# ESA-PRL/planning-path_planning

Measured on NVIDIA B200. Metric: plans_per_s, higher is better.
Workload: dtype f64

## Files before the change

### planning-path_planning_b200/csrc/dymu_fim.cu

```cuda
#include <cooperative_groups.h>
#include <stdlib.h>

#include "dymu_ctx.cuh"

namespace
{
constexpr int TILE = kTile;
static_assert(TILE == 32, "4 x 4 blocks of 8 x 8 cells");
constexpr int ROUNDS = 6;
constexpr int WARPS = 16;
constexpr int THREADS = 32 * WARPS;
constexpr int BX = TILE / 8;
constexpr int BY = TILE / 8;
constexpr int PITCH = TILE + 4;
constexpr int CPT = TILE * TILE / THREADS;
constexpr int MIN_CTAS = 2;
constexpr int SWEEP_CAP = 2 * TILE;
constexpr size_t SMEM = sizeof(double) * ((TILE + 2) * PITCH + TILE * PITCH);
constexpr size_t SMEM_ANISO = sizeof(double) * ((TILE + 2) * PITCH + 4 * TILE * PITCH);

constexpr uint32_t kHaloTop = 1u, kHaloBottom = 2u, kHaloLeft = 4u, kHaloRight = 8u, kFull = 16u,
                   kResume = 32u;

struct Params
{
    double* T;
    size_t slot_stride;
    const double* C;
    uint32_t pitch, rows, ntx, nty, nprob;
    uint32_t* list0;
    uint32_t* list1;
    uint32_t* list2;
    uint32_t* flag0;
    uint32_t* flag1;
    uint32_t* flag2;
    unsigned long long* key0;
    unsigned long long* key1;
    unsigned long long* key2;
    unsigned long long* gmin;
    uint32_t* dsave;
    unsigned long long* cta_trace;
    uint32_t cta_trace_phases;
    uint32_t* ctrl;
    unsigned long long* stats;
    int max_outer;
    int outer0;
    double band;
    unsigned long long* tmax;
    double* xout;
    size_t xld;
    uint32_t xnx, xny;
    int xminus1;
    const uint32_t* stop_flag;
    uint32_t stop_value;
    const double* A;
    size_t a_stride;
};
constexpr unsigned long long kExported = 0xFFFFFFFFFFFFFFFFull;

__device__ __forceinline__ uint32_t ld_volatile_u32(const uint32_t* p)
{
    return *reinterpret_cast<const volatile uint32_t*>(p);
}
__device__ __forceinline__ unsigned long long ld_volatile_u64(const unsigned long long* p)
{
    return *reinterpret_cast<const volatile unsigned long long*>(p);
}
__device__ __forceinline__ void smem_or(uint32_t* p, uint32_t v)
{
    asm volatile("red.shared.or.b32 [%0], %1;" ::"r"((uint32_t)__cvta_generic_to_shared(p)), "r"(v) : "memory");
}
constexpr unsigned long long kNoKey = 0xFFFFFFFFFFFFFFFFull;
__device__ __forceinline__ unsigned long long key_of(double v)
{
    return (unsigned long long)__double_as_longlong(v);
}

__device__ __noinline__ bool barrier_spin(const uint32_t* counter, uint32_t target,
                                          unsigned long long* abort_flag)
{
    uint32_t polls = 0;
    unsigned long long t0 = 0;
    while (ld_volatile_u32(counter) < target)
    {
        if ((++polls & 0x3FFFu) == 0)
        {
            if (ld_volatile_u64(abort_flag)) return false;
            unsigned long long now;
            asm volatile("mov.u64 %0, %%globaltimer;" : "=l"(now));
            if (t0 == 0) t0 = now;
            else if (now - t0 > 8000000000ull)
            {
                *abort_flag = 1ull;
                __threadfence();
                return false;
            }
        }
    }
    return true;
}

__device__ __forceinline__ bool grid_barrier(uint32_t* counter, uint32_t& phase, unsigned long long* abort_flag,
                                             uint32_t* ok)
{
    __syncthreads();
    if (threadIdx.x == 0)
    {
        __threadfence();
        uint32_t target = (phase + 1) * gridDim.x;
        atomicAdd(counter, 1u);
        *ok = barrier_spin(counter, target, abort_flag) ? 1u : 0u;
        __threadfence();
    }
    phase++;
    __syncthreads();
    return *ok != 0;
}

__device__ __forceinline__ void grid_barrier_arrive(uint32_t* counter, uint32_t phase, uint32_t* order)
{
    __syncthreads();
    if (threadIdx.x == 0)
    {
        __threadfence();
        *order = atomicAdd(counter, 1u) - phase * gridDim.x;
    }
}
__device__ __forceinline__ bool grid_barrier_wait(uint32_t* counter, uint32_t& phase, unsigned long long* abort_flag,
                                                  uint32_t* ok)
{
    if (threadIdx.x == 0)
    {
        uint32_t target = (phase + 1) * gridDim.x;
        *ok = barrier_spin(counter, target, abort_flag) ? 1u : 0u;
        __threadfence();
    }
    phase++;
    __syncthreads();
    return *ok != 0;
}

template <int MODE> __device__ __forceinline__ double outside_value()
{
    return MODE == 1 ? 0.0 : DYMU_INF;
}

__device__ __forceinline__ double min_nn(double a, double b)
{
    long long x = __double_as_longlong(a), y = __double_as_longlong(b);
    return __longlong_as_double(x < y ? x : y);
}
__device__ __forceinline__ double max_nn(double a, double b)
{
    long long x = __double_as_longlong(a), y = __double_as_longlong(b);
    return __longlong_as_double(x > y ? x : y);
}

template <int MODE>
__device__ __forceinline__ bool relax(double tc, double tl, double tr, double tu, double td,
                                      double c, double cc2 , double& out)
{
    if (MODE == 0)
    {
        const double Tx = min_nn(tl, tr), Ty = min_nn(td, tu);
        const double d = Tx - Ty;
        const bool two = fabs(d) < c;
        const double t2 = (Tx + Ty + dymu_sqrt_normal(cc2 - (d * d))) * 0.5;
        const double t1 = min_nn(Tx, Ty) + c;
        const double Tn = two ? t2 : t1;
        out = Tn;
        return Tn < tc;
    }
    else
    {
        const double Ry = max_nn(tu, td), Rx = max_nn(tl, tr);
        const double Sx = 1 - Rx, Sy = 1 - Ry;
        const double d = Sx - Sy;
        const bool target = c < DYMU_INF;
        const bool two = fabs(d) < c;
        double arg = (two && target) ? (2 * (c * c) - (d * d)) : 1.0;
        asm volatile("" : "+d"(arg));
        const double s2 = (Sx + Sy + dymu_sqrt_normal(arg)) / 2;
        const double s1 = fmin(Sx, Sy) + c;
        const double S = two ? s2 : s1;
        const double R = fmax(1 - S, 0.0);
        out = R;
        return target && (R > 0) && (R > tc);
    }
}

__device__ __forceinline__ double aniso_pair(double Th, double ah, double Tv, double av)
{
    const double d = Th - Tv;
    const double ah2 = ah * ah, av2 = av * av;
    const double s = ah2 + av2;
    const bool valid = (d > -ah) && (d < av) && (s < DYMU_INF);
    const double t = ((av2 * Th + ah2 * Tv) + (ah * av) * dymu_sqrt_normal(s - d * d)) / s;
    return valid ? t : DYMU_INF;
}

__device__ __forceinline__ bool relax_aniso(double tc, double txm, double txp, double tym, double typ,
                                            const double* ac, int ps, double& out)
{
    const double axm = ac[0], axp = ac[ps], aym = ac[2 * ps], ayp = ac[3 * ps];
    double Tn = min_nn(min_nn(txm + axm, txp + axp), min_nn(tym + aym, typ + ayp));
    Tn = min_nn(Tn, min_nn(aniso_pair(txm, axm, tym, aym), aniso_pair(txm, axm, typ, ayp)));
    Tn = min_nn(Tn, min_nn(aniso_pair(txp, axp, tym, aym), aniso_pair(txp, axp, typ, ayp)));
    out = Tn;
    return Tn < tc;
}

template <int MODE>
__global__ void __launch_bounds__(THREADS, MIN_CTAS) k_fim(Params p)
{
    constexpr int P = PITCH;
    extern __shared__ __align__(16) unsigned char smem_raw[];
    double* Ts = reinterpret_cast<double*>(smem_raw);
    double* Cs = Ts + (TILE + 2) * P;
    __shared__ uint32_t s_post[2][WARPS];
    __shared__ uint32_t s_m0;
    __shared__ uint32_t edge_mask;
    __shared__ uint32_t s_tile;
    __shared__ unsigned long long s_emin[5];
    __shared__ uint32_t s_tmax;
    __shared__ uint32_t s_xtile;
    __shared__ uint32_t s_xorder;
    __shared__ uint32_t s_bar_ok;

    const int tid = threadIdx.x, lane = tid & 31, warp = tid >> 5;
    const uint32_t tiles_per_prob = p.ntx * p.nty;
    constexpr int c_off = (TILE + 1) * P - 1;
    __shared__ uint2 s_wake[THREADS];
    double* cell1;
    int to_second;
    uint32_t my_bit;
    {
        const int lx = lane & 7, ly = lane >> 3;
        const bool upper_is_red = (lx & 1) == 0;
        to_second = upper_is_red ? P : -P;
        asm volatile("" : "+r"(to_second));
        const int bx = warp & 3, by = warp >> 2;
        int off = (by * 8 + 2 * ly + (upper_is_red ? 0 : 1) + 1) * P + bx * 8 + lx + 1;
        asm volatile("" : "+r"(off));
        cell1 = Ts + off;
        my_bit = 1u << warp;
        const uint32_t bitL = bx > 0 ? my_bit >> 1 : 0x40000u, bitR = bx < BX - 1 ? my_bit << 1 : 0x80000u;
        const uint32_t bitU = by > 0 ? my_bit >> 4 : 0x10000u, bitD = by < BY - 1 ? my_bit << 4 : 0x20000u;
        const uint32_t side = (lx == 0 ? bitL : 0u) | (lx == 7 ? bitR : 0u);
        const uint32_t w_upper = my_bit | side | (ly == 0 ? bitU : 0u);
        const uint32_t w_lower = my_bit | side | (ly == 3 ? bitD : 0u);
        s_wake[tid] = upper_is_red ? make_uint2(w_upper, w_lower) : make_uint2(w_lower, w_upper);
    }
    auto sel3 = [](uint32_t* a, uint32_t* b, uint32_t* c, int k) { return k == 0 ? a : (k == 1 ? b : c); };
    auto sel3k = [](unsigned long long* a, unsigned long long* b, unsigned long long* c, int k) {
        return k == 0 ? a : (k == 1 ? b : c);
    };
    auto deliver_tile = [&](uint32_t t) {
        const uint32_t ty = t / p.ntx, tx = t - ty * p.ntx;
#pragma unroll
        for (int k = 0; k < CPT; ++k)
        {
            const int e = tid + k * THREADS;
            const uint32_t gy = ty * TILE + e / TILE, gx = tx * TILE + e % TILE;
            if (gx < p.xnx && gy < p.xny)
            {
                double v = __ldcg(&p.T[(size_t)gy * p.pitch + gx]);
                if (p.xminus1 && v == DYMU_INF) v = -1.0;
                p.xout[(size_t)gy * p.xld + gx] = v;
            }
        }
    };
    uint32_t phase = 0;
    unsigned long long n_tiles = 0, n_visits = 0, n_deferred = 0, n_inner = 0;
    uint32_t n_written = 0;
#ifdef DYMU_FIM_PROFILE
    long long pc_fetch = 0, pc_load = 0, pc_sweep = 0, pc_store = 0, pc_barrier = 0, pc_t = clock64();
#define PC_MARK(acc) { long long now__ = clock64(); acc += now__ - pc_t; pc_t = now__; }
    unsigned long long tl_fetch = 0, tl_load = 0, tl_sweep = 0, tl_store = 0, tl_tiles = 0, tl_start = 0;
#define GT(var) { unsigned long long g__; asm volatile("mov.u64 %0, %%globaltimer;" : "=l"(g__)); var = g__; }
#else
#define PC_MARK(acc)
#endif
    int outer = p.outer0;
    bool converged = false;

    for (; outer < p.outer0 + p.max_outer; ++outer)
    {
        const int cur = outer % 3, nxt = (outer + 1) % 3, old = (outer + 2) % 3;
        const uint32_t n_active = ld_volatile_u32(&p.ctrl[kCtrlCount + cur]);
        if (n_active == 0)
        {
            converged = true;
            break;
        }
        if (p.stop_flag)
        {
            const uint32_t stop_at = ld_volatile_u32(&p.ctrl[kCtrlStopAt]);
            if (stop_at != 0 && stop_at <= (uint32_t)outer + 1u) break;
        }
#ifdef DYMU_FIM_PROFILE
        if (tid == 0) { GT(tl_start) tl_fetch = tl_load = tl_sweep = tl_store = tl_start; tl_tiles = 0; }
#endif
        uint32_t* list_cur = sel3(p.list0, p.list1, p.list2, cur);
        uint32_t* list_nxt = sel3(p.list0, p.list1, p.list2, nxt);
        uint32_t* flag_cur = sel3(p.flag0, p.flag1, p.flag2, cur);
        uint32_t* flag_nxt = sel3(p.flag0, p.flag1, p.flag2, nxt);
        unsigned long long* key_cur = sel3k(p.key0, p.key1, p.key2, cur);
        unsigned long long* key_nxt = sel3k(p.key0, p.key1, p.key2, nxt);
        unsigned long long limit = kNoKey;
        {
            const unsigned long long gm = ld_volatile_u64(&p.gmin[cur]);
            const double lim = __longlong_as_double((long long)gm) + p.band;
            if (gm != kNoKey && lim < DYMU_INF) limit = key_of(lim);
        }

        bool first_fetch = true;
        for (;;)
        {
            __syncthreads();
            if (tid == 0)
            {
                uint32_t t = 0xffffffffu;
                for (;;)
                {
                    uint32_t idx;
                    if (first_fetch)
                    {
                        idx = blockIdx.x;
                        first_fetch = false;
                    }
                    else
                    {
                        if (n_active <= gridDim.x) break;
                        idx = gridDim.x + atomicAdd(&p.ctrl[kCtrlCursor + cur], 1u);
                    }
                    if (idx >= n_active) break;
                    const uint32_t cand = ld_volatile_u32(&list_cur[idx]);
                    const unsigned long long k = ld_volatile_u64(&key_cur[cand]);
                    if (k <= limit)
                    {
                        t = cand;
                        break;
                    }
                    const uint32_t bits = ld_volatile_u32(&flag_cur[cand]);
                    flag_cur[cand] = 0;
                    key_cur[cand] = kNoKey;
                    atomicMin(&key_nxt[cand], k);
                    atomicMin(&p.gmin[nxt], k);
                    if (atomicOr(&flag_nxt[cand], bits) == 0)
                        list_nxt[atomicAdd(&p.ctrl[kCtrlCount + nxt], 1u)] = cand;
                    n_deferred++;
                }
                s_tile = t;
            }
            __syncthreads();
            PC_MARK(pc_fetch)
            const uint32_t tile_id = s_tile;
#ifdef DYMU_FIM_PROFILE
            if (tid == 0 && tile_id != 0xffffffffu && tl_tiles == 0) GT(tl_fetch)
#endif
            if (tile_id == 0xffffffffu) break;
            const uint32_t prob = tile_id / tiles_per_prob;
            const uint32_t trem = tile_id - prob * tiles_per_prob;
            const uint32_t ty = trem / p.ntx, tx = trem - ty * p.ntx;
            const uint32_t why = ld_volatile_u32(&flag_cur[tile_id]);
            double* Tg = p.T + (size_t)prob * p.slot_stride + (size_t)ty * TILE * p.pitch
                         + (size_t)tx * TILE;
            const double* Cg = p.C + (size_t)ty * TILE * p.pitch + (size_t)tx * TILE;

            static_assert(4 * TILE <= THREADS, "one halo cell per thread");
            double hv = outside_value<MODE>();
            int hslot = -1;
            if (tid < 4 * TILE)
            {
                const int side = tid / TILE, q = tid % TILE;
                const double* src = nullptr;
                if (side == 0)
                {
                    if (ty > 0) src = &Tg[-(ptrdiff_t)p.pitch + q];
                    hslot = q + 1;
                }
                else if (side == 1)
                {
                    if (ty + 1 < p.nty) src = &Tg[(size_t)TILE * p.pitch + q];
                    hslot = (TILE + 1) * P + q + 1;
                }
                else if (side == 2)
                {
                    if (tx > 0) src = &Tg[(size_t)q * p.pitch - 1];
                    hslot = (q + 1) * P;
                }
                else
                {
                    if (tx + 1 < p.ntx) src = &Tg[(size_t)q * p.pitch + TILE];
                    hslot = (q + 1) * P + TILE + 1;
                }
                if (src) hv = __ldcg(src);
            }
            double told[CPT];
#pragma unroll
            for (int k = 0; k < CPT; ++k)
            {
                int e = tid + k * THREADS;
                int y = e / TILE, x = e % TILE;
                double v = __ldcg(&Tg[(size_t)y * p.pitch + x]);
                told[k] = v;
                Ts[(y + 1) * P + x + 1] = v;
                if constexpr (MODE == 2)
                {
#pragma unroll
                    for (int q = 0; q < 4; ++q)
                        Cs[q * TILE * P + y * P + x] =
                            __ldg(&p.A[q * p.a_stride + (size_t)(ty * TILE + y) * p.pitch + tx * TILE + x]);
                }
                else
                    Cs[y * P + x] = __ldg(&Cg[(size_t)y * p.pitch + x]);
            }
            if (hslot >= 0) Ts[hslot] = hv;
            if (tid == 0)
            {
                uint32_t m0 = 0;
                if (why & kResume) m0 |= p.dsave[tile_id];
                if (why & kFull) m0 = 0xffffu;
                if (why & kHaloTop) m0 |= 0x000Fu;
                if (why & kHaloBottom) m0 |= 0xF000u;
                if (why & kHaloLeft) m0 |= 0x1111u;
                if (why & kHaloRight) m0 |= 0x8888u;
                s_m0 = m0;
                flag_cur[tile_id] = 0;
                key_cur[tile_id] = kNoKey;
            }
            if (tid == 0)
            {
                edge_mask = 0;
                s_tmax = 0;
            }
            if (tid < 5) s_emin[tid] = kNoKey;
            __syncthreads();
            PC_MARK(pc_load)
#ifdef DYMU_FIM_PROFILE
            if (tid == 0 && tl_tiles == 0) GT(tl_load)
#endif

            int it = 0;
            uint32_t visits = 0;
            uint32_t m = s_m0;
            uint32_t edges_acc = 0;
            const double cA = cell1[c_off], cB = cell1[to_second + c_off];
            const double qA = 2 * (cA * cA), qB = 2 * (cB * cB);
            auto sweep = [&](uint32_t* post) -> uint32_t {
                uint32_t contrib = 0;
                if (m & my_bit)
                {
                    double* a = cell1;
                    double* b = a + to_second;
                    uint2 wake = s_wake[tid];
                    asm volatile("" : "+r"(wake.x), "+r"(wake.y));
                    uint32_t woke = 0;
#pragma unroll
                    for (int round = 0; round < ROUNDS; ++round)
                    {
                        double tA = a[0];
                        const double lA = a[-1], rA = a[1], uA = a[-P], dA = a[P];
                        asm volatile("" : "+d"(tA));
                        double nA, nB;
                        bool chA;
                        if constexpr (MODE == 2)
                            chA = relax_aniso(tA, lA, rA, uA, dA, a + c_off, TILE * P, nA);
                        else
                            chA = relax<MODE>(tA, lA, rA, uA, dA, cA, qA, nA);
                        if (chA) a[0] = nA;
                        __syncwarp();
                        const double tB = b[0];
                        const double lB = b[-1], rB = b[1], uB = b[-P], dB = b[P];
                        bool chB;
                        if constexpr (MODE == 2)
                            chB = relax_aniso(tB, lB, rB, uB, dB, b + c_off, TILE * P, nB);
                        else
                            chB = relax<MODE>(tB, lB, rB, uB, dB, cB, qB, nB);
                        if (chB) b[0] = nB;
                        woke |= (chA ? wake.x : 0u) | (chB ? wake.y : 0u);
                        visits += 2;
                        if (round + 1 < ROUNDS)
                        {
                            if (!__any_sync(0xffffffffu, chA || chB)) break;
                        }
                    }
                    contrib = __reduce_or_sync(0xffffffffu, woke);
                }
                edges_acc |= contrib >> 16;
                if (lane == 0) post[warp] = contrib & 0xffffu;
                __syncthreads();
                ++it;
                return __reduce_or_sync(0xffffffffu, post[lane & (WARPS - 1)]);
            };
            for (;;)
            {
                if (m == 0 || it >= SWEEP_CAP) break;
                m = sweep(s_post[0]);
                if (m == 0 || it >= SWEEP_CAP) break;
                m = sweep(s_post[1]);
            }
            if (edges_acc && lane == 0) smem_or(&edge_mask, edges_acc);
            n_visits += visits;
            const int more = (m != 0);
            if (more && tid == 0) p.dsave[tile_id] = m;
            PC_MARK(pc_sweep)
#ifdef DYMU_FIM_PROFILE
            if (tid == 0 && tl_tiles == 0) GT(tl_sweep)
#endif

            uint32_t vmax = 0;
            {
                unsigned long long kmin[5] = {kNoKey, kNoKey, kNoKey, kNoKey, kNoKey};
                bool any = false;
#pragma unroll
                for (int k = 0; k < CPT; ++k)
                {
                    int e = tid + k * THREADS;
                    int y = e / TILE, x = e % TILE;
                    double v = Ts[(y + 1) * P + x + 1];
                    if (MODE != 1 && p.tmax && Cs[y * P + x] < DYMU_INF)
                        vmax = max(vmax, (uint32_t)(key_of(v) >> 32) + 1u);
                    if (v != told[k])
                    {
                        n_written++;
                        __stcg(&Tg[(size_t)y * p.pitch + x], v);
                        if (MODE != 1)
                        {
                            const unsigned long long kb = key_of(v);
                            any = true;
                            if (y == 0 && v < Ts[x + 1]) kmin[0] = min(kmin[0], kb);
                            if (y == TILE - 1 && v < Ts[(TILE + 1) * P + x + 1]) kmin[1] = min(kmin[1], kb);
                            if (x == 0 && v < Ts[(y + 1) * P]) kmin[2] = min(kmin[2], kb);
                            if (x == TILE - 1 && v < Ts[(y + 1) * P + TILE + 1]) kmin[3] = min(kmin[3], kb);
                            if (more) kmin[4] = min(kmin[4], kb);
                        }
                    }
                }
                if (MODE != 1 && __any_sync(0xffffffffu, any))
                {
#pragma unroll
                    for (int q = 0; q < 5; ++q)
                    {
                        const uint32_t hi = (uint32_t)(kmin[q] >> 32), lo = (uint32_t)kmin[q];
                        const uint32_t mhi = __reduce_min_sync(0xffffffffu, hi);
                        const uint32_t mlo = __reduce_min_sync(0xffffffffu, hi == mhi ? lo : 0xffffffffu);
                        const unsigned long long r = ((unsigned long long)mhi << 32) | mlo;
                        if (lane == 0 && r != kNoKey) atomicMin(&s_emin[q], r);
                    }
                }
            }
            if (MODE != 1 && p.tmax)
            {
                vmax = __reduce_max_sync(0xffffffffu, vmax);
                if (lane == 0 && vmax) atomicMax(&s_tmax, vmax);
            }
            __syncthreads();
            if (tid < 5)
            {
                uint32_t target = 0xffffffffu, bit = 0;
                uint32_t em = edge_mask;
                if (MODE != 1)
                    em = (s_emin[0] != kNoKey ? 1u : 0u) | (s_emin[1] != kNoKey ? 2u : 0u)
                         | (s_emin[2] != kNoKey ? 4u : 0u) | (s_emin[3] != kNoKey ? 8u : 0u);
                if (tid == 0 && (em & 1u) && ty > 0) { target = tile_id - p.ntx; bit = kHaloBottom; }
                if (tid == 1 && (em & 2u) && ty + 1 < p.nty) { target = tile_id + p.ntx; bit = kHaloTop; }
                if (tid == 2 && (em & 4u) && tx > 0) { target = tile_id - 1; bit = kHaloRight; }
                if (tid == 3 && (em & 8u) && tx + 1 < p.ntx) { target = tile_id + 1; bit = kHaloLeft; }
                if (tid == 4 && more) { target = tile_id; bit = kResume; }
                if (MODE != 1 && tid == 4 && p.tmax) p.tmax[tile_id] = (unsigned long long)s_tmax << 32;
                if (target != 0xffffffffu)
                {
                    unsigned long long kb = (MODE != 1) ? s_emin[tid] : 0ull;
                    if (kb == kNoKey) kb = 0ull;
                    atomicMin(&key_nxt[target], kb);
                    atomicMin(&p.gmin[nxt], kb);
                    if (atomicOr(&flag_nxt[target], bit) == 0)
                    {
                        uint32_t pos = atomicAdd(&p.ctrl[kCtrlCount + nxt], 1u);
                        list_nxt[pos] = target;
                    }
                }
            }
            n_tiles++;
            n_inner += (unsigned long long)it;
            PC_MARK(pc_store)
#ifdef DYMU_FIM_PROFILE
            if (tid == 0) { GT(tl_store) tl_tiles++; }
#endif
        }
        PC_MARK(pc_fetch)
#ifdef DYMU_FIM_PROFILE
        if (tid == 0 && p.cta_trace && (uint32_t)outer < p.cta_trace_phases)
        {
            unsigned long long tl_arrive; GT(tl_arrive)
            unsigned long long* o = p.cta_trace + ((size_t)outer * gridDim.x + blockIdx.x) * 8;
            o[0] = tl_start; o[1] = tl_fetch; o[2] = tl_load; o[3] = tl_sweep; o[4] = tl_store;
            o[5] = tl_arrive; o[6] = tl_tiles; o[7] = n_active;
        }
#endif
        if (blockIdx.x == 0 && tid == 0)
        {
            if (p.stop_flag && ld_volatile_u32(&p.ctrl[kCtrlStopAt]) == 0 && ld_volatile_u32(p.stop_flag) >= p.stop_value)
                p.ctrl[kCtrlStopAt] = (uint32_t)outer + 2u;
            p.ctrl[kCtrlCount + old] = 0;
            p.ctrl[kCtrlCursor + old] = 0;
            p.gmin[old] = kNoKey;
        }
        if (MODE != 1 && p.xout)
        {
            const unsigned long long gm = ld_volatile_u64(&p.gmin[cur]);
            grid_barrier_arrive(&p.ctrl[kCtrlBarrier], phase, &s_xorder);
            if (tid == 0) s_xtile = 0xffffffffu;
            __syncthreads();
            const uint32_t order = s_xorder, sharers = max(gridDim.x / 2u, 1u);
            if (order < sharers)
            {
                const uint32_t per = (tiles_per_prob + sharers - 1) / sharers;
                const uint32_t t_end = min((order + 1) * per, tiles_per_prob);
                for (uint32_t t = order * per + tid; t < t_end; t += THREADS)
                    if (ld_volatile_u64(&p.tmax[t]) < gm && atomicCAS(&s_xtile, 0xffffffffu, t) == 0xffffffffu)
                        p.tmax[t] = kExported;
                __syncthreads();
                const uint32_t xt = s_xtile;
                if (xt != 0xffffffffu)
                {
                    deliver_tile(xt);
                    if (tid == 0) atomicAdd(&p.stats[kStatDelivered], 1ull);
                }
            }
            if (!grid_barrier_wait(&p.ctrl[kCtrlBarrier], phase, &p.stats[kStatAbort], &s_bar_ok)) break;
        }
        else if (!grid_barrier(&p.ctrl[kCtrlBarrier], phase, &p.stats[kStatAbort], &s_bar_ok))
            break;
        PC_MARK(pc_barrier)
    }
#ifdef DYMU_FIM_PROFILE
    if (tid == 0)
    {
        atomicAdd(&p.stats[kStatCycFetch], (unsigned long long)pc_fetch);
        atomicAdd(&p.stats[kStatCycLoad], (unsigned long long)pc_load);
        atomicAdd(&p.stats[kStatCycSweep], (unsigned long long)pc_sweep);
        atomicAdd(&p.stats[kStatCycStore], (unsigned long long)pc_store);
        atomicAdd(&p.stats[kStatCycBarrier], (unsigned long long)pc_barrier);
    }
#endif

    if (lane == 0 && n_visits) atomicAdd(&p.stats[kStatVisits], n_visits);
    {
        const uint32_t w = __reduce_add_sync(0xffffffffu, n_written);
        if (lane == 0 && w) atomicAdd(&p.stats[kStatWritten], (unsigned long long)w);
    }
    if (tid == 0)
    {
        if (n_tiles) atomicAdd(&p.stats[kStatTiles], n_tiles);
        if (n_deferred) atomicAdd(&p.stats[kStatDeferred], n_deferred);
        if (n_inner) atomicAdd(&p.stats[kStatSweeps], n_inner);
        if (blockIdx.x == 0)
        {
            p.stats[kStatPhases] = (unsigned long long)(outer - p.outer0);
            p.stats[kStatConverged] = converged ? 1ull : 0ull;
        }
    }
}


__global__ void __launch_bounds__(512) k_deliver_rest(const double* T, uint32_t pitch, uint32_t ntx, uint32_t nty,
                                                      unsigned long long* tmax, double* xout, size_t xld,
                                                      uint32_t xnx, uint32_t xny, int xminus1,
                                                      unsigned long long* stats)
{
    if (ld_volatile_u64(&stats[kStatConverged]) == 0) return;
    const uint32_t total = ntx * nty;
    for (uint32_t t = blockIdx.x; t < total; t += gridDim.x)
    {
        if (ld_volatile_u64(&tmax[t]) == kExported) continue;
        const uint32_t ty = t / ntx, tx = t - ty * ntx;
        for (uint32_t e = threadIdx.x; e < TILE * TILE; e += blockDim.x)
        {
            const uint32_t gy = ty * TILE + e / TILE, gx = tx * TILE + e % TILE;
            if (gx < xnx && gy < xny)
            {
                double v = __ldcg(&T[(size_t)gy * pitch + gx]);
                if (xminus1 && v == DYMU_INF) v = -1.0;
                xout[(size_t)gy * xld + gx] = v;
            }
        }
    }
}

__global__ void k_seed(double* T, size_t slot_stride, uint32_t pitch, uint32_t ntx, uint32_t nty,
                       int tile, const uint32_t* goal_ij, uint32_t n, const uint8_t* obst, uint32_t* list0,
                       uint32_t* flag0, unsigned long long* key0, unsigned long long* gmin,
                       uint32_t* ctrl, unsigned long long* stats)
{
    if (blockIdx.x != 0 || threadIdx.x != 0) return;
    uint32_t n_seeded = 0;
    for (uint32_t q = 0; q < n; ++q)
    {
        uint32_t gi = goal_ij[2 * q], gj = goal_ij[2 * q + 1];
        if (obst && obst[(size_t)gj * pitch + gi])
        {
            stats[kStatGoalObstacle]++;
            continue;
        }
        T[(size_t)q * slot_stride + (size_t)gj * pitch + gi] = 0.0;
        uint32_t tile_id = q * ntx * nty + (gj / tile) * ntx + gi / tile;
        flag0[tile_id] = kFull;
        key0[tile_id] = 0ull;
        list0[n_seeded++] = tile_id;
    }
    ctrl[kCtrlCount] = n_seeded;
    if (n_seeded) gmin[0] = 0ull;
}

__global__ void k_seed_all(uint32_t n, uint32_t* list0, uint32_t* flag0, unsigned long long* key0,
                           unsigned long long* gmin, uint32_t* ctrl)
{
    uint32_t q = blockIdx.x * blockDim.x + threadIdx.x;
    if (q >= n) return;
    list0[q] = q;
    flag0[q] = kFull;
    key0[q] = 0ull;
    if (q == 0)
    {
        ctrl[kCtrlCount] = n;
        gmin[0] = 0ull;
    }
}

__global__ void k_seed_rows(uint32_t ntx, const uint32_t* tile_rows, uint32_t n_tile_rows, uint32_t* list0,
                            uint32_t* flag0, unsigned long long* key0, unsigned long long* gmin,
                            uint32_t* ctrl)
{
    uint32_t n = n_tile_rows * ntx;
    uint32_t q = blockIdx.x * blockDim.x + threadIdx.x;
    if (q >= n) return;
    uint32_t tile_id = tile_rows[q / ntx] * ntx + q % ntx;
    flag0[tile_id] = kFull;
    key0[tile_id] = 0ull;
    list0[q] = tile_id;
    if (q == 0)
    {
        ctrl[kCtrlCount] = n;
        gmin[0] = 0ull;
    }
}

__global__ void k_seed_rows_add(uint32_t ntx, const uint32_t* tile_rows, uint32_t n_tile_rows, uint32_t* list,
                                uint32_t* flag, unsigned long long* key, unsigned long long* gmin_cur,
                                uint32_t* count_cur, unsigned long long seed_key)
{
    uint32_t n = n_tile_rows * ntx;
    uint32_t q = blockIdx.x * blockDim.x + threadIdx.x;
    if (q >= n) return;
    uint32_t tile_id = tile_rows[q / ntx] * ntx + q % ntx;
    atomicMin(&key[tile_id], seed_key);
    if (atomicOr(&flag[tile_id], kFull) == 0) list[atomicAdd(count_cur, 1u)] = tile_id;
    if (q == 0) atomicMin(gmin_cur, seed_key);
}

__global__ void k_import_rows_min(double* T, uint32_t pitch, uint32_t nx, uint32_t j0, uint32_t n_rows,
                                  const double* src, int* changed, unsigned long long* min_lowered)
{
    size_t total = (size_t)nx * n_rows;
    size_t stride = (size_t)gridDim.x * blockDim.x;
    int any = 0;
    unsigned long long lowest = kNoKey;
    for (size_t k = (size_t)blockIdx.x * blockDim.x + threadIdx.x; k < total; k += stride)
    {
        uint32_t r = (uint32_t)(k / nx), i = (uint32_t)(k % nx);
        double v = src[k];
        double* t = &T[(size_t)(j0 + r) * pitch + i];
        if (v < *t)
        {
            *t = v;
            any = 1;
            lowest = min(lowest, key_of(v));
        }
    }
    if (__any_sync(0xffffffffu, any))
    {
        for (int o = 16; o > 0; o >>= 1) lowest = min(lowest, __shfl_xor_sync(0xffffffffu, lowest, o));
        if ((threadIdx.x & 31) == 0)
        {
            *changed = 1;
            atomicMin(min_lowered, lowest);
        }
    }
}

template <int MODE> int launch_fim(dymu_ctx* ctx, Params& prm, size_t total_tiles)
{
    constexpr size_t smem = MODE == 2 ? SMEM_ANISO : SMEM;
    int per_sm = 0;
    DYMU_CUDA_TRY(ctx, cudaFuncSetAttribute(k_fim<MODE>,
                                            cudaFuncAttributeMaxDynamicSharedMemorySize,
                                            (int)smem));
    DYMU_CUDA_TRY(ctx, cudaOccupancyMaxActiveBlocksPerMultiprocessor(
                           &per_sm, k_fim<MODE>, THREADS, smem));
    if (per_sm < 1) DYMU_FAIL(ctx, DYMU_ERR_CUDA, "FIM kernel does not fit on an SM");
    size_t grid = (size_t)per_sm * ctx->sm_count;
    if (grid > total_tiles) grid = total_tiles;
    if (grid < 1) grid = 1;
    void* args[] = {&prm};
    DYMU_CUDA_TRY(ctx, cudaLaunchCooperativeKernel((void*)k_fim<MODE>, dim3((unsigned)grid),
                                                   dim3(THREADS), args,
                                                   smem, ctx->stream));
    ctx->launches++;
    return DYMU_OK;
}
}

int dymu_internal_fim_alloc(dymu_ctx* ctx, dymu_fim_work* w, size_t capacity)
{
    dymu_internal_fim_free(w);
    w->capacity = capacity;
    for (int k = 0; k < 3; ++k)
    {
        DYMU_CUDA_TRY(ctx, cudaMalloc((void**)&w->list[k], capacity * sizeof(uint32_t)));
        DYMU_CUDA_TRY(ctx, cudaMalloc((void**)&w->flag[k], capacity * sizeof(uint32_t)));
        DYMU_CUDA_TRY(ctx, cudaMemsetAsync(w->flag[k], 0, capacity * sizeof(uint32_t), ctx->stream));
        DYMU_CUDA_TRY(ctx, cudaMalloc((void**)&w->key[k], capacity * sizeof(unsigned long long)));
        DYMU_CUDA_TRY(ctx, cudaMemsetAsync(w->key[k], 0xFF, capacity * sizeof(unsigned long long),
                                           ctx->stream));
    }
    DYMU_CUDA_TRY(ctx, cudaMalloc((void**)&w->ctrl, kCtrlWords * sizeof(uint32_t)));
    DYMU_CUDA_TRY(ctx, cudaMalloc((void**)&w->gmin, 4 * sizeof(unsigned long long)));
    DYMU_CUDA_TRY(ctx, cudaMalloc((void**)&w->dsave, capacity * sizeof(uint32_t)));
    DYMU_CUDA_TRY(ctx, cudaMemsetAsync(w->dsave, 0, capacity * sizeof(uint32_t), ctx->stream));
    DYMU_CUDA_TRY(ctx, cudaMalloc((void**)&w->stats, kStatWords * sizeof(unsigned long long)));
    w->rot = 0;
    w->pending = false;
    w->unclean = false;
    return DYMU_OK;
}

void dymu_internal_fim_free(dymu_fim_work* w)
{
    for (int k = 0; k < 3; ++k)
    {
        if (w->list[k]) cudaFree(w->list[k]);
        if (w->flag[k]) cudaFree(w->flag[k]);
        if (w->key[k]) cudaFree(w->key[k]);
        w->list[k] = w->flag[k] = nullptr;
        w->key[k] = nullptr;
    }
    if (w->ctrl) cudaFree(w->ctrl);
    if (w->gmin) cudaFree(w->gmin);
    if (w->dsave) cudaFree(w->dsave);
    w->gmin = nullptr;
    w->dsave = nullptr;
    if (w->stats) cudaFree(w->stats);
    w->ctrl = nullptr;
    w->stats = nullptr;
    w->capacity = 0;
}

int dymu_internal_fim_configure(dymu_ctx* ctx)
{
    int dev_coop = 0;
    DYMU_CUDA_TRY(ctx, cudaDeviceGetAttribute(&dev_coop, cudaDevAttrCooperativeLaunch, ctx->device));
    if (!dev_coop) DYMU_FAIL(ctx, DYMU_ERR_NODEVICE, "device lacks cooperative launch");
    ctx->fim_band = 1.0 / 0.0;
    return DYMU_OK;
}

int dymu_internal_fim_clear(dymu_ctx* ctx, dymu_fim_work* w)
{
    DYMU_TRY(dymu_internal_settle_delivery(ctx));
    if (w->unclean)
    {
        for (int k = 0; k < 3; ++k)
        {
            DYMU_CUDA_TRY(ctx, cudaMemsetAsync(w->flag[k], 0, w->capacity * sizeof(uint32_t), ctx->stream));
            DYMU_CUDA_TRY(ctx, cudaMemsetAsync(w->key[k], 0xFF, w->capacity * sizeof(unsigned long long),
                                               ctx->stream));
        }
        DYMU_CUDA_TRY(ctx, cudaMemsetAsync(w->dsave, 0, w->capacity * sizeof(uint32_t), ctx->stream));
    }
    DYMU_CUDA_TRY(ctx, cudaMemsetAsync(w->ctrl, 0, kCtrlWords * sizeof(uint32_t), ctx->stream));
    DYMU_CUDA_TRY(ctx, cudaMemsetAsync(w->gmin, 0xFF, 4 * sizeof(unsigned long long), ctx->stream));
    DYMU_CUDA_TRY(ctx, cudaMemsetAsync(w->stats, 0, kStatWords * sizeof(unsigned long long), ctx->stream));
    w->rot = 0;
    w->pending = false;
    return DYMU_OK;
}

int dymu_internal_fim_seed_all(dymu_ctx* ctx, dymu_fim_work* w, uint32_t n_tiles)
{
    DYMU_TRY(dymu_internal_fim_clear(ctx, w));
    k_seed_all<<<dymu_div_up(n_tiles, 128), 128, 0, ctx->stream>>>(n_tiles, w->list[0], w->flag[0], w->key[0],
                                                                    w->gmin, w->ctrl);
    ctx->launches++;
    DYMU_CUDA_TRY(ctx, cudaGetLastError());
    return DYMU_OK;
}

dymu_fim_launch dymu_internal_global_launch(dymu_ctx* ctx, uint32_t nprob)
{
    dymu_fim_launch L;
    L.T = ctx->T; L.slot_stride = (size_t)ctx->pitch * ctx->rows; L.C = ctx->ceff;
    L.pitch = ctx->pitch; L.rows = ctx->rows; L.ntx = ctx->ntx; L.nty = ctx->nty; L.nprob = nprob;
    L.work = &ctx->work;
    L.mode = ctx->aniso_n ? 2 : 0;
    L.A = ctx->aniso_n ? ctx->dircost : nullptr;
    L.band = ctx->aniso_n ? ctx->aniso_band : ctx->fim_band;
    return L;
}

int dymu_internal_fim_run(dymu_ctx* ctx, const dymu_fim_launch& L, dymu_solve_stats* stats)
{
    dymu_fim_work* w = L.work;
    Params prm;
    prm.T = L.T;
    prm.slot_stride = L.slot_stride;
    prm.C = L.C;
    prm.pitch = L.pitch;
    prm.rows = L.rows;
    prm.ntx = L.ntx;
    prm.nty = L.nty;
    prm.nprob = L.nprob;
    prm.list0 = w->list[0]; prm.list1 = w->list[1]; prm.list2 = w->list[2];
    prm.flag0 = w->flag[0]; prm.flag1 = w->flag[1]; prm.flag2 = w->flag[2];
    prm.key0 = w->key[0]; prm.key1 = w->key[1]; prm.key2 = w->key[2];
    prm.gmin = w->gmin;
    prm.dsave = w->dsave;
    prm.cta_trace = nullptr;
    prm.cta_trace_phases = 0;
    unsigned long long* d_cta_trace = nullptr;
    const uint32_t cta_trace_phases = 400;
    const char* cta_trace_path = getenv("DYMU_FIM_CTA_TRACE");
#ifdef DYMU_FIM_PROFILE
    if (cta_trace_path && L.mode == 0)
    {
        size_t bytes = (size_t)cta_trace_phases * 1024 * 8 * 8;
        DYMU_CUDA_TRY(ctx, cudaMalloc((void**)&d_cta_trace, bytes));
        DYMU_CUDA_TRY(ctx, cudaMemsetAsync(d_cta_trace, 0, bytes, ctx->stream));
        prm.cta_trace = d_cta_trace;
        prm.cta_trace_phases = cta_trace_phases;
    }
#endif
    prm.ctrl = w->ctrl;
    prm.stats = w->stats;
    prm.stop_flag = L.stop_flag;
    prm.stop_value = L.stop_value;
    prm.tmax = nullptr;
    prm.xout = nullptr;
    prm.xld = 0;
    prm.xnx = ctx->nx;
    prm.xny = ctx->ny;
    prm.xminus1 = ctx->export_xform == DYMU_XFORM_INF_TO_MINUS1;
    if (L.mode != 1 && L.nprob == 1 && L.T == ctx->T && ctx->tile_tmax && (L.track_final || L.export_now))
    {
        prm.tmax = ctx->tile_tmax;
        if (L.export_now && ctx->export_dev)
        {
            prm.xout = ctx->export_dev;
            prm.xld = ctx->export_ld;
// ... 578 lines not shown
```

Baseline: 108.2.

## Batch deferred-tile requeues and move wakeup atomics off the critical path

Deferred (over-band) tiles are now buffered in shared memory and flushed in warp-wide batches, with ballot-aggregated list appends and warp-reduced gmin updates, instead of being requeued one at a time with serial atomics by thread 0. Neighbour wakeups for a finished tile are deferred to warp 1 at the top of the next fetch iteration, so they overlap with tile fetching instead of running serially at the end of the tile. The first tile's list entry and gmin are prefetched at phase start, and a late key check lets even the first-fetched tile be deferred. This adds shared-memory state and more control-flow complexity, and it risks ordering subtleties around when wakeups become visible.

```diff
diff --git a/planning-path_planning_b200/csrc/dymu_fim.cu b/planning-path_planning_b200/csrc/dymu_fim.cu
--- a/planning-path_planning_b200/csrc/dymu_fim.cu
+++ b/planning-path_planning_b200/csrc/dymu_fim.cu
@@ -57,6 +57,8 @@
     size_t a_stride;
 };
 constexpr unsigned long long kExported = 0xFFFFFFFFFFFFFFFFull;
+constexpr int kDeferCap = 64;
+constexpr uint32_t kNoTile = 0xffffffffu, kFlushTile = 0xfffffffeu;
 
 __device__ __forceinline__ uint32_t ld_volatile_u32(const uint32_t* p)
 {
@@ -221,6 +223,10 @@
     __shared__ uint32_t s_m0;
     __shared__ uint32_t edge_mask;
     __shared__ uint32_t s_tile;
+    __shared__ uint32_t s_woke;
+    __shared__ unsigned long long s_limit;
+    __shared__ uint32_t s_ndef, s_dtile[kDeferCap], s_dbits[kDeferCap];
+    __shared__ unsigned long long s_dkey[kDeferCap];
     __shared__ unsigned long long s_emin[5];
     __shared__ uint32_t s_tmax;
     __shared__ uint32_t s_xtile;
@@ -271,7 +277,8 @@
         }
     };
     uint32_t phase = 0;
-    unsigned long long n_tiles = 0, n_visits = 0, n_deferred = 0, n_inner = 0;
+    unsigned long long n_tiles = 0, n_visits = 0, n_inner = 0;
+    uint32_t n_deferred = 0;
     uint32_t n_written = 0;
 #ifdef DYMU_FIM_PROFILE
     long long pc_fetch = 0, pc_load = 0, pc_sweep = 0, pc_store = 0, pc_barrier = 0, pc_t = clock64();
@@ -287,7 +294,15 @@
     for (; outer < p.outer0 + p.max_outer; ++outer)
     {
         const int cur = outer % 3, nxt = (outer + 1) % 3, old = (outer + 2) % 3;
+        uint32_t* list_cur = sel3(p.list0, p.list1, p.list2, cur);
         const uint32_t n_active = ld_volatile_u32(&p.ctrl[kCtrlCount + cur]);
+        unsigned long long gm = kNoKey;
+        uint32_t cand0 = 0;
+        if (tid == 0)
+        {
+            gm = ld_volatile_u64(&p.gmin[cur]);
+            cand0 = ld_volatile_u32(&list_cur[blockIdx.x]);
+        }
         if (n_active == 0)
         {
             converged = true;
@@ -301,55 +316,126 @@
 #ifdef DYMU_FIM_PROFILE
         if (tid == 0) { GT(tl_start) tl_fetch = tl_load = tl_sweep = tl_store = tl_start; tl_tiles = 0; }
 #endif
-        uint32_t* list_cur = sel3(p.list0, p.list1, p.list2, cur);
         uint32_t* list_nxt = sel3(p.list0, p.list1, p.list2, nxt);
         uint32_t* flag_cur = sel3(p.flag0, p.flag1, p.flag2, cur);
         uint32_t* flag_nxt = sel3(p.flag0, p.flag1, p.flag2, nxt);
         unsigned long long* key_cur = sel3k(p.key0, p.key1, p.key2, cur);
         unsigned long long* key_nxt = sel3k(p.key0, p.key1, p.key2, nxt);
-        unsigned long long limit = kNoKey;
-        {
-            const unsigned long long gm = ld_volatile_u64(&p.gmin[cur]);
+        if (tid == 0)
+        {
             const double lim = __longlong_as_double((long long)gm) + p.band;
-            if (gm != kNoKey && lim < DYMU_INF) limit = key_of(lim);
-        }
-
+            s_limit = (gm != kNoKey && lim < DYMU_INF) ? key_of(lim) : kNoKey;
+            s_woke = 0xffffffffu;
+            s_ndef = 0;
+        }
+
+        auto send_wakeups = [&](uint32_t t, bool t_more) {
+            const uint32_t trem = t - (t / tiles_per_prob) * tiles_per_prob;
+            const uint32_t ty = trem / p.ntx, tx = trem - ty * p.ntx;
+            uint32_t target = 0xffffffffu, bit = 0;
+            uint32_t em = edge_mask;
+            if (MODE != 1)
+                em = (s_emin[0] != kNoKey ? 1u : 0u) | (s_emin[1] != kNoKey ? 2u : 0u)
+                     | (s_emin[2] != kNoKey ? 4u : 0u) | (s_emin[3] != kNoKey ? 8u : 0u);
+            if (lane == 0 && (em & 1u) && ty > 0) { target = t - p.ntx; bit = kHaloBottom; }
+            if (lane == 1 && (em & 2u) && ty + 1 < p.nty) { target = t + p.ntx; bit = kHaloTop; }
+            if (lane == 2 && (em & 4u) && tx > 0) { target = t - 1; bit = kHaloRight; }
+            if (lane == 3 && (em & 8u) && tx + 1 < p.ntx) { target = t + 1; bit = kHaloLeft; }
+            if (lane == 4 && t_more) { target = t; bit = kResume; }
+            unsigned long long kb = kNoKey;
+            if (target != 0xffffffffu)
+            {
+                kb = (MODE != 1) ? s_emin[lane] : 0ull;
+                if (kb == kNoKey) kb = 0ull;
+                atomicMin(&key_nxt[target], kb);
+            }
+            const uint32_t hi = (uint32_t)(kb >> 32), lo = (uint32_t)kb;
+            const uint32_t mhi = __reduce_min_sync(0xffffffffu, hi);
+            const uint32_t mlo = __reduce_min_sync(0xffffffffu, hi == mhi ? lo : 0xffffffffu);
+            const unsigned long long kmin = ((unsigned long long)mhi << 32) | mlo;
+            if (lane == 0 && kmin != kNoKey) atomicMin(&p.gmin[nxt], kmin);
+            if (target != 0xffffffffu && atomicOr(&flag_nxt[target], bit) == 0)
+                list_nxt[atomicAdd(&p.ctrl[kCtrlCount + nxt], 1u)] = target;
+        };
+        auto defer_entry = [&](uint32_t t, unsigned long long k, uint32_t bits) {
+            flag_cur[t] = 0;
+            key_cur[t] = kNoKey;
+            const uint32_t n = s_ndef;
+            s_dtile[n] = t;
+            s_dkey[n] = k;
+            s_dbits[n] = bits;
+            s_ndef = n + 1;
+            n_deferred++;
+        };
+        auto flush_deferred = [&]() {
+            const uint32_t n = s_ndef;
+            for (uint32_t b = 0; b < n; b += 32)
+            {
+                const uint32_t i = b + lane;
+                const bool on = i < n;
+                const uint32_t t = on ? s_dtile[i] : 0u;
+                const unsigned long long k = on ? s_dkey[i] : kNoKey;
+                if (on) atomicMin(&key_nxt[t], k);
+                const uint32_t hi = (uint32_t)(k >> 32), lo = (uint32_t)k;
+                const uint32_t mhi = __reduce_min_sync(0xffffffffu, hi);
+                const uint32_t mlo = __reduce_min_sync(0xffffffffu, hi == mhi ? lo : 0xffffffffu);
+                if (lane == 0) atomicMin(&p.gmin[nxt], ((unsigned long long)mhi << 32) | mlo);
+                const bool app = on && atomicOr(&flag_nxt[t], s_dbits[i]) == 0;
+                const uint32_t bal = __ballot_sync(0xffffffffu, app);
+                if (bal)
+                {
+                    uint32_t base = 0;
+                    if (lane == 0) base = atomicAdd(&p.ctrl[kCtrlCount + nxt], (uint32_t)__popc(bal));
+                    base = __shfl_sync(0xffffffffu, base, 0);
+                    if (app) list_nxt[base + __popc(bal & ((1u << lane) - 1u))] = t;
+                }
+            }
+            __syncwarp();
+            if (lane == 0) s_ndef = 0;
+        };
         bool first_fetch = true;
         for (;;)
         {
             __syncthreads();
+            if (warp == 1)
+            {
+                const uint32_t w = s_woke;
+                if (w != 0xffffffffu)
+                {
+                    send_wakeups(w & 0x7fffffffu, (w >> 31) != 0);
+                    __syncwarp();
+                    if (lane == 0) s_woke = 0xffffffffu;
+                }
+            }
             if (tid == 0)
             {
-                uint32_t t = 0xffffffffu;
-                for (;;)
+                uint32_t t = kNoTile;
+                if (first_fetch)
                 {
-                    uint32_t idx;
-                    if (first_fetch)
+                    first_fetch = false;
+                    if (blockIdx.x < n_active) t = cand0;
+                }
+                else if (n_active > gridDim.x)
+                {
+                    for (;;)
                     {
-                        idx = blockIdx.x;
-                        first_fetch = false;
+                        if (s_ndef == kDeferCap)
+                        {
+                            t = kFlushTile;
+                            break;
+                        }
+                        const uint32_t idx = gridDim.x + atomicAdd(&p.ctrl[kCtrlCursor + cur], 1u);
+                        if (idx >= n_active) break;
+                        const uint32_t cand = ld_volatile_u32(&list_cur[idx]);
+                        const unsigned long long k = ld_volatile_u64(&key_cur[cand]);
+                        const uint32_t bits = ld_volatile_u32(&flag_cur[cand]);
+                        if (k <= s_limit)
+                        {
+                            t = cand;
+                            break;
+                        }
+                        defer_entry(cand, k, bits);
                     }
-                    else
-                    {
-                        if (n_active <= gridDim.x) break;
-                        idx = gridDim.x + atomicAdd(&p.ctrl[kCtrlCursor + cur], 1u);
-                    }
-                    if (idx >= n_active) break;
-                    const uint32_t cand = ld_volatile_u32(&list_cur[idx]);
-                    const unsigned long long k = ld_volatile_u64(&key_cur[cand]);
-                    if (k <= limit)
-                    {
-                        t = cand;
-                        break;
-                    }
-                    const uint32_t bits = ld_volatile_u32(&flag_cur[cand]);
-                    flag_cur[cand] = 0;
-                    key_cur[cand] = kNoKey;
-                    atomicMin(&key_nxt[cand], k);
-                    atomicMin(&p.gmin[nxt], k);
-                    if (atomicOr(&flag_nxt[cand], bits) == 0)
-                        list_nxt[atomicAdd(&p.ctrl[kCtrlCount + nxt], 1u)] = cand;
-                    n_deferred++;
                 }
                 s_tile = t;
             }
@@ -357,13 +443,24 @@
             PC_MARK(pc_fetch)
             const uint32_t tile_id = s_tile;
 #ifdef DYMU_FIM_PROFILE
-            if (tid == 0 && tile_id != 0xffffffffu && tl_tiles == 0) GT(tl_fetch)
+            if (tid == 0 && tile_id < kFlushTile && tl_tiles == 0) GT(tl_fetch)
 #endif
-            if (tile_id == 0xffffffffu) break;
+            if (tile_id >= kFlushTile)
+            {
+                if (warp == 0 && s_ndef != 0) flush_deferred();
+                if (tile_id == kNoTile) break;
+                continue;
+            }
             const uint32_t prob = tile_id / tiles_per_prob;
             const uint32_t trem = tile_id - prob * tiles_per_prob;
             const uint32_t ty = trem / p.ntx, tx = trem - ty * p.ntx;
-            const uint32_t why = ld_volatile_u32(&flag_cur[tile_id]);
+            unsigned long long tkey = 0;
+            uint32_t why = 0;
+            if (tid == 0)
+            {
+                tkey = ld_volatile_u64(&key_cur[tile_id]);
+                why = ld_volatile_u32(&flag_cur[tile_id]);
+            }
             double* Tg = p.T + (size_t)prob * p.slot_stride + (size_t)ty * TILE * p.pitch
                          + (size_t)tx * TILE;
             const double* Cg = p.C + (size_t)ty * TILE * p.pitch + (size_t)tx * TILE;
@@ -417,7 +514,12 @@
                     Cs[y * P + x] = __ldg(&Cg[(size_t)y * p.pitch + x]);
             }
             if (hslot >= 0) Ts[hslot] = hv;
-            if (tid == 0)
+            if (tid == 0 && tkey > s_limit)
+            {
+                defer_entry(tile_id, tkey, why);
+                s_m0 = 0xffffffffu;
+            }
+            else if (tid == 0)
             {
                 uint32_t m0 = 0;
                 if (why & kResume) m0 |= p.dsave[tile_id];
@@ -437,6 +539,7 @@
             }
             if (tid < 5) s_emin[tid] = kNoKey;
             __syncthreads();
+            if (s_m0 == 0xffffffffu) continue;
             PC_MARK(pc_load)
 #ifdef DYMU_FIM_PROFILE
             if (tid == 0 && tl_tiles == 0) GT(tl_load)
@@ -557,32 +660,8 @@
                 if (lane == 0 && vmax) atomicMax(&s_tmax, vmax);
             }
             __syncthreads();
-            if (tid < 5)
-            {
-                uint32_t target = 0xffffffffu, bit = 0;
-                uint32_t em = edge_mask;
-                if (MODE != 1)
-                    em = (s_emin[0] != kNoKey ? 1u : 0u) | (s_emin[1] != kNoKey ? 2u : 0u)
-                         | (s_emin[2] != kNoKey ? 4u : 0u) | (s_emin[3] != kNoKey ? 8u : 0u);
-                if (tid == 0 && (em & 1u) && ty > 0) { target = tile_id - p.ntx; bit = kHaloBottom; }
-                if (tid == 1 && (em & 2u) && ty + 1 < p.nty) { target = tile_id + p.ntx; bit = kHaloTop; }
-                if (tid == 2 && (em & 4u) && tx > 0) { target = tile_id - 1; bit = kHaloRight; }
-                if (tid == 3 && (em & 8u) && tx + 1 < p.ntx) { target = tile_id + 1; bit = kHaloLeft; }
-                if (tid == 4 && more) { target = tile_id; bit = kResume; }
-                if (MODE != 1 && tid == 4 && p.tmax) p.tmax[tile_id] = (unsigned long long)s_tmax << 32;
-                if (target != 0xffffffffu)
-                {
-                    unsigned long long kb = (MODE != 1) ? s_emin[tid] : 0ull;
-                    if (kb == kNoKey) kb = 0ull;
-                    atomicMin(&key_nxt[target], kb);
-                    atomicMin(&p.gmin[nxt], kb);
-                    if (atomicOr(&flag_nxt[target], bit) == 0)
-                    {
-                        uint32_t pos = atomicAdd(&p.ctrl[kCtrlCount + nxt], 1u);
-                        list_nxt[pos] = target;
-                    }
-                }
-            }
+            if (MODE != 1 && tid == 0 && p.tmax) p.tmax[tile_id] = (unsigned long long)s_tmax << 32;
+            if (tid == 0) s_woke = tile_id | (more ? 0x80000000u : 0u);
             n_tiles++;
             n_inner += (unsigned long long)it;
             PC_MARK(pc_store)
@@ -655,7 +734,7 @@
     if (tid == 0)
     {
         if (n_tiles) atomicAdd(&p.stats[kStatTiles], n_tiles);
-        if (n_deferred) atomicAdd(&p.stats[kStatDeferred], n_deferred);
+        if (n_deferred) atomicAdd(&p.stats[kStatDeferred], (unsigned long long)n_deferred);
         if (n_inner) atomicAdd(&p.stats[kStatSweeps], n_inner);
         if (blockIdx.x == 0)
         {
```

Result: no change. 108.8, median of 6 (+0.5%).
